# zhaoweicai/mscnn

Hardware: AMD Instinct MI355X
Metric: images/sec mscnn-7s-576 KITTI-car inference (higher is better)
Workload: dtype f32

## Files before the change

include/mscnn_hip.h:

```cpp
#ifndef MSCNN_HIP_H_
#define MSCNN_HIP_H_

#include <stddef.h>
#include <stdint.h>

#if defined(__GNUC__)
#define MSCNN_API __attribute__((visibility("default")))
#else
#define MSCNN_API
#endif

#ifdef __cplusplus
extern "C" {
#endif

typedef enum {
  MSCNN_OK = 0,
  MSCNN_ERR_BAD_ARG = 1,
  MSCNN_ERR_HIP = 2,
  MSCNN_ERR_WORKSPACE = 3,
  MSCNN_ERR_UNSUPPORTED = 4
} mscnn_status;

MSCNN_API const char* mscnn_last_error(void);
MSCNN_API const char* mscnn_version(void);

typedef struct mscnn_conv_plan mscnn_conv_plan;

typedef enum {
  MSCNN_CONV_ALGO_AUTO = 0,
  MSCNN_CONV_ALGO_DIRECT = 1,
  MSCNN_CONV_ALGO_WINO_F2 = 2,
  MSCNN_CONV_ALGO_WINO_F3 = 3,
  MSCNN_CONV_ALGO_F16 = 4,
  MSCNN_CONV_ALGO_WINO_F3_X3 = 5,
  MSCNN_CONV_ALGO_WINO_F4 = 6
} mscnn_conv_algo;

typedef struct {
  int N, Cin, H, W;
  int Cout, Kh, Kw;
  int pad_h, pad_w, stride_h, stride_w, group;
  int relu;
  int algo;
  int tune_variant, tune_grid, tune_flags;
} mscnn_conv_desc;

MSCNN_API int mscnn_conv2d_plan_create(const mscnn_conv_desc* desc, mscnn_conv_plan** plan_out);
MSCNN_API void mscnn_conv2d_plan_destroy(mscnn_conv_plan* plan);
MSCNN_API size_t mscnn_conv2d_packed_weight_bytes(const mscnn_conv_plan* plan);
MSCNN_API size_t mscnn_conv2d_workspace_bytes(const mscnn_conv_plan* plan);
MSCNN_API const char* mscnn_conv2d_plan_kernel(const mscnn_conv_plan* plan);
MSCNN_API double mscnn_conv2d_plan_flops(const mscnn_conv_plan* plan);
MSCNN_API const char* mscnn_conv2d_plan_dtype(const mscnn_conv_plan* plan);
MSCNN_API double mscnn_conv2d_plan_executed_flops(const mscnn_conv_plan* plan);
MSCNN_API int mscnn_conv2d_plan_plane_columns(const mscnn_conv_plan* plan, int* cols, int n);
MSCNN_API int mscnn_conv2d_plan_set_profiling(mscnn_conv_plan* plan, int on);
MSCNN_API int mscnn_conv2d_plan_stage_ms(const mscnn_conv_plan* plan, float ms_out[3]);
#define MSCNN_AMAX_SLOTS 1024
MSCNN_API int mscnn_conv2d_plan_publishes_amax(const mscnn_conv_plan* plan);
MSCNN_API int mscnn_conv2d_plan_set_amax_io(mscnn_conv_plan* plan, const uint32_t* in_bound, uint32_t* out_amax);
MSCNN_API int mscnn_conv2d_plan_set_batch(mscnn_conv_plan* plan, int N);
MSCNN_API unsigned long long mscnn_conv2d_plan_weight_layout(const mscnn_conv_plan* plan);
MSCNN_API int mscnn_conv2d_pack_weights(const mscnn_conv_plan* plan, const float* w, float* packed, void* stream);
MSCNN_API int mscnn_conv2d_fwd_f32(const mscnn_conv_plan* plan, const float* x, const float* w, const float* packed,
                         const float* bias, float* y, void* workspace, size_t workspace_bytes, void* stream);
MSCNN_API int mscnn_conv2d_plan_can_pool(const mscnn_conv_plan* plan);
MSCNN_API int mscnn_conv2d_fwd_pool_f32(const mscnn_conv_plan* plan, const float* x, const float* w, const float* packed,
                              const float* bias, float* y, float* y_pool, void* workspace, size_t workspace_bytes,
                              void* stream);

MSCNN_API int mscnn_relu_fwd_f32(const float* x, float* y, size_t count, float negative_slope, void* stream);

MSCNN_API int mscnn_pool_out_dim(int in, int kernel, int pad, int stride);
MSCNN_API int mscnn_pool2d_fwd_f32(const float* x, float* y, int N, int C, int H, int W, int kernel_h, int kernel_w,
                         int pad_h, int pad_w, int stride_h, int stride_w, int method, void* stream);

MSCNN_API int mscnn_inner_product_fwd_f32(const float* x, const float* w, const float* bias, float* y,
                                int M, int N, int K, int relu, void* stream);
MSCNN_API void mscnn_debug_inner_product_rows(int rows);

MSCNN_API int mscnn_inner_product_wg_supported(int M, int N, int K);
MSCNN_API size_t mscnn_inner_product_wg_packed_bytes(int N, int K);
MSCNN_API size_t mscnn_inner_product_wg_workspace_bytes(int M, int N, int K);
MSCNN_API int mscnn_inner_product_wg_pack(const float* w, float* wt, int N, int K, void* stream);
MSCNN_API int mscnn_inner_product_wg_fwd(const float* x, const float* wt, const float* bias, float* y, int M, int N, int K, int relu,
                                         void* workspace, size_t workspace_bytes, void* stream);
MSCNN_API unsigned long long mscnn_wgemm_handoff_event(void);
MSCNN_API void mscnn_wgemm_force_whole_tiles(int on);
// ... 197 lines not shown
```

mscnn_amd/csrc/conv.hip:

```cpp
#include "common.h"
#include <cstring>
#include "headconv.h"
#include "winograd.h"
#include "wino_x3.h"
#include "wgemm.h"
#include "roipool_wino.h"
#include "wino33_device.h"
#include "conv_c3.h"
#include "wconv.h"
#include "wf2conv.h"
#include "x3_device.h"
#include <new>
#include <type_traits>

namespace {

typedef float f32x16 __attribute__((ext_vector_type(16)));
typedef _Float16 f16x8 __attribute__((ext_vector_type(8)));

struct IgemmArgs {
  const float* x; const float* wp; const float* bias; float* y; float* ws;
  int N, Cin, H, W, Cout, Ho, Wo, pad_h, pad_w;
  int MT, NTH, NTW, NT, KI, G, relu;
  int xcd_map;
// ... 1139 lines not shown
  const int genv = tune_env("MSCNN_TUNE_GRID", d.tune_grid);
  long G = genv > 0 ? genv : ((k.BM == 128 && k.BN == 128 && k.KH == 3 && k.variant != 200) || k.variant == 201 || k.variant == 4 ? 768 : 512);
  if (tiles * p->KI / 4 < G) G = tiles * p->KI / 4;
  if (G < 1) G = 1;
  if (!genv && tiles >= 2 * G) {
    const long tops[3] = {k.variant == 106 ? 1024 : 0, (k.KH == 1 && k.BN == 128 && k.CK < 64) ? 768 : 0, G};
    bool found = false;
    for (int c = 0; c < 3 && !found; ++c)
      for (long g2 = tops[c]; g2 > 0 && g2 >= tops[c] - tops[c] / (k.KH == 3 ? 50 : 16) && g2 * 2 <= tiles; --g2)
        if (tiles % g2 == 0) { G = g2; found = true; break; }
  }
  if (!genv && k.KH == 1 && k.variant >= 101 && tiles >= 256 && tiles <= 768) G = tiles;
  p->G = (int)G;
  p->full_q = (int)(tiles / G);
  p->total_iters = (tiles - (long)p->full_q * G) * p->KI;
  p->packed_bytes = (size_t)p->MT * p->KI * k.KH * k.KW * k.CK * k.BM * ((k.variant >= 200 && k.variant <= 202) ? sizeof(_Float16) : sizeof(float));
  p->ws_bytes = (size_t)p->G * kSlabsPerWg * k.BM * k.BN * sizeof(float);
  if (k.variant == 210) {
    p->x3d_hdr_off = (size_t)p->MT * p->KI * k.KH * k.KW * k.CK * k.BM * 2 * sizeof(_Float16);
    p->packed_bytes = p->x3d_hdr_off + 8192;
    p->x3d_slots_off = p->ws_bytes;
    p->ws_bytes += 4096;
  }
  if (k.KH == 3 && k.KW == 3 && k.BM == 64 && k.CK == 8 && k.RH == 0 && (k.variant == 0 || k.variant == 1) && p->MT == 1 && d.pad_h == 1 &&
      d.pad_w == 1 && !(tune_env("MSCNN_TUNE_FLAGS", d.tune_flags) & 32768)) {
    if (mscnn::wconv_plan(d.N, d.Cin, d.H, d.W, d.Cout, d.tune_variant == 402, &p->wc) && p->wc.packed_bytes == p->packed_bytes) p->wc_use = true;
  }
  if (p->entry >= 0 && k.KH == 3 && k.KW == 3 && k.BM == 64 && k.RH == 0 && (k.variant == 0 || k.variant == 1) && p->MT == 1 && d.pad_h == 1 && d.pad_w == 1 &&
      d.stride_h == 1 && d.stride_w == 1 && d.group == 1 && tune_env("MSCNN_CONV_ALGO", d.algo) == MSCNN_CONV_ALGO_AUTO &&
      !(tune_env("MSCNN_TUNE_FLAGS", d.tune_flags) & 65536) && mscnn::wf2_plan(d.N, d.Cin, d.H, d.W, d.Cout, &p->wf) &&
      (p->wf.tiles >= 512 || d.tune_variant == 403)) {
    p->wf_use = true;
    p->wc_use = false;
    p->packed_bytes = p->wf.packed_bytes;
    p->ws_bytes = 0;
  }
}

extern "C" int mscnn_conv2d_plan_create(const mscnn_conv_desc* desc, mscnn_conv_plan** plan_out) {
  MSCNN_REQUIRE(desc && plan_out, "conv plan: null pointer");
  const mscnn_conv_desc& d = *desc;
  MSCNN_REQUIRE(d.N >= 0 && d.Cin > 0 && d.H > 0 && d.W > 0 && d.Cout > 0 && d.Kh > 0 && d.Kw > 0, "conv plan: bad shape");
  MSCNN_REQUIRE(d.stride_h > 0 && d.stride_w > 0 && d.pad_h >= 0 && d.pad_w >= 0 && d.group > 0, "conv plan: bad params");
  MSCNN_REQUIRE(d.Cin % d.group == 0 && d.Cout % d.group == 0, "conv plan: channels not divisible by group");
  MSCNN_REQUIRE(d.H + 2 * d.pad_h >= d.Kh && d.W + 2 * d.pad_w >= d.Kw, "conv plan: kernel larger than padded input");
  mscnn_conv_plan* p = new (std::nothrow) mscnn_conv_plan();
  MSCNN_REQUIRE(p, "conv plan: out of memory");
  p->d = d;
  plan_shape(p);
  *plan_out = p;
  return MSCNN_OK;
}

extern "C" void mscnn_conv2d_plan_destroy(mscnn_conv_plan* plan) { delete plan; }
extern "C" size_t mscnn_conv2d_packed_weight_bytes(const mscnn_conv_plan* p) { return p ? p->packed_bytes : 0; }
extern "C" size_t mscnn_conv2d_workspace_bytes(const mscnn_conv_plan* p) { return p ? p->ws_bytes : 0; }
extern "C" const char* mscnn_conv2d_plan_kernel(const mscnn_conv_plan* p) {
  if (!p) return "";
  if (p->x3h.rows) return "head_gemm_shiftadd_x3f16";
  if (p->hg) return p->hg_kw ? "head_kwfold_shiftadd_f32" : "head_gemm_shiftadd_f32";
  if (p->head.entry >= 0) return head_kernel_name(p->head);
  if (p->x3.BM) return p->x3.BM == 256 ? "winograd_f3x3_3x3_x3f16_256" : "winograd_f3x3_3x3_x3f16_128";
  if (p->wino) return p->wino_m == 4 ? "winograd_f4x4_3x3" : p->wino_m == 3 ? "winograd_f3x3_3x3" : "winograd_f2x2_3x3";
  if (p->c3) return mscnn::c3_kernel_name();
  if (p->wf_use) return mscnn::wf2_kernel_name();
  if (p->wc_use) return mscnn::wconv_kernel_name();
// ... 38 lines not shown
  const double planes = (double)((p->wino_m + 2) * (p->wino_m + 2)) * (p->x3.BM ? 3.0 : 1.0);
  return 2.0 * planes * d.Cout * d.Cin * ((double)d.N * p->tiles_h * p->tiles_w);
}
extern "C" int mscnn_conv2d_plan_plane_columns(const mscnn_conv_plan* p, int* cols, int n) {
  if (!p || (!p->wino && !p->x3.BM)) return 0;
  const int planes = (p->wino_m + 2) * (p->wino_m + 2);
  for (int i = 0; i < planes && i < n && cols; ++i) cols[i] = p->ragged ? p->wg.cols[i] : p->d.N * p->tiles_h * p->tiles_w;
  return planes;
}
extern "C" long mscnn_debug_wgemm_schedule(const mscnn_conv_plan* p, int whole_tiles, int* rows, long max_rows, int info[8]) {
  if (!p || !p->wino || !p->use_wg) return -1;
  if (info) {
    const int v[8] = {p->wg.tiles, p->wg.MT, p->wg.KI, p->wg.G, p->wg.full_q, p->wg.P, p->wg.BN, p->wg.ragged};
    for (int i = 0; i < 8; ++i) info[i] = v[i];
  }
  return mscnn::wgemm_debug_schedule(p->wg, whole_tiles, rows, max_rows);
}
extern "C" int mscnn_conv2d_plan_set_profiling(mscnn_conv_plan* p, int on) {
  MSCNN_REQUIRE(p, "conv plan: null");
  p->profiling = on != 0;
  p->ev_valid = false;
  if (p->profiling)
    for (hipEvent_t& e : p->ev)
      if (!e) MSCNN_HIP_TRY(hipEventCreate(&e));
  return MSCNN_OK;
}
extern "C" int mscnn_conv2d_plan_stage_ms(const mscnn_conv_plan* p, float ms_out[3]) {
  MSCNN_REQUIRE(p && ms_out, "conv plan: null");
  ms_out[0] = ms_out[1] = ms_out[2] = 0.f;
  MSCNN_REQUIRE(p->profiling && p->ev_valid, "conv plan: no profiled forward yet (mscnn_conv2d_plan_set_profiling)");
  MSCNN_HIP_TRY(hipEventSynchronize(p->ev[3]));
  for (int i = 0; i < 3; ++i) MSCNN_HIP_TRY(hipEventElapsedTime(&ms_out[i], p->ev[i], p->ev[i + 1]));
  return MSCNN_OK;
}
extern "C" int mscnn_conv2d_plan_publishes_amax(const mscnn_conv_plan* p) {
  return p && !p->x3h.rows && (p->x3.BM || (p->wino && p->wino_m >= 3) || p->c3 ||
               (!p->wino && p->head.entry < 0 && p->entry >= 0 && !p->wc_use && !p->wf_use && !(kTable[p->entry].variant >= 200 && kTable[p->entry].variant <= 202))) ? 1 : 0;
}
extern "C" int mscnn_conv2d_plan_set_amax_io(mscnn_conv_plan* p, const uint32_t* in_bound, uint32_t* out_amax) {
  MSCNN_REQUIRE(p, "conv plan: null");
  if (out_amax && !mscnn_conv2d_plan_publishes_amax(p)) {
    set_error("conv plan: kernel %s does not publish max |y|", mscnn_conv2d_plan_kernel(p));
    return MSCNN_ERR_UNSUPPORTED;
  }
  p->amax_in = in_bound;
  p->amax_out = out_amax;
  return MSCNN_OK;
}
extern "C" int mscnn_conv2d_plan_set_batch(mscnn_conv_plan* p, int N) {
  MSCNN_REQUIRE(p && N >= 0, "conv plan: bad batch");
  p->d.N = N;
  plan_shape(p);
  return MSCNN_OK;
}

extern "C" int mscnn_conv2d_pack_weights(const mscnn_conv_plan* p, const float* w, float* packed, void* stream) {
  MSCNN_REQUIRE(p, "conv pack: null plan");
  MSCNN_REQUIRE_ALIGNED(packed, 16, "conv pack: packed");
  if (p->x3h.rows) {
    MSCNN_REQUIRE(w && packed, "conv pack: null pointer");
    return x3_head_pack(p->x3h, w, packed, as_stream(stream));
  }
  if (p->hg) {
    MSCNN_REQUIRE(w && packed, "conv pack: null pointer");
    float* wprime = reinterpret_cast<float*>(reinterpret_cast<unsigned char*>(packed) + p->hg->packed_bytes);
    if (p->hg_kw) {
// ... 386 lines not shown
```

mscnn_amd/csrc/wf2conv.h:

```cpp
#pragma once
#include <hip/hip_runtime.h>
#include <cstddef>

namespace mscnn {

struct Wf2Plan {
  int N, Cin, H, W;
  int NTH, NTW, KI, tiles;
  int cus;
  size_t packed_bytes;
};

bool wf2_plan(int N, int Cin, int H, int W, int Cout, Wf2Plan* out);
const char* wf2_kernel_name();
int wf2_pack(const Wf2Plan& p, const float* w, float* packed, hipStream_t st);
int wf2_launch(const Wf2Plan& p, const float* x, const float* packed, const float* bias, float* y, float* y_pool, int relu, hipStream_t st);

}
```

mscnn_amd/csrc/wf2conv.hip:

```cpp
#include "wf2conv.h"
#include "common.h"
#include <type_traits>

namespace {

typedef float f32x4 __attribute__((ext_vector_type(4)));

struct Wf2Args {
  const float* x; const float* up; const float* bias; float* y; float* yp;
  int N, Cin, H, W, NTH, NTW, KI, relu, tiles;
  int dG_w, dG_h, dG_n;
  unsigned x_bytes;
};

#ifndef WF2_ABL
#define WF2_ABL 0
#endif
#ifdef WF2_TRACE
__device__ unsigned long long g_wf2_trace[2 * 32 * 8];
#define WF2_STAMP(k) do { if (slot == 0 && (wave & 3) == 0 && lane == 0 && u >= 8 && u < 40) g_wf2_trace[((wave >> 2) * 32 + (u - 8)) * 8 + (k)] = __builtin_amdgcn_s_memtime(); } while (0)
#else
#define WF2_STAMP(k) do { } while (0)
#endif
constexpr int TR = 4, TC = 16, NT = TR * TC;
// ... 14 lines not shown
#pragma unroll
  for (int b = 0; b < 3; ++b) {
    const float g0 = g[b], g1 = g[3 + b], g2 = g[6 + b];
    t[0][b] = g0; t[1][b] = 0.5f * (g0 + g1 + g2); t[2][b] = 0.5f * (g0 - g1 + g2); t[3][b] = g2;
  }
#pragma unroll
  for (int a = 0; a < 4; ++a) {
    const float u0 = t[a][0], u1 = 0.5f * (t[a][0] + t[a][1] + t[a][2]), u2 = 0.5f * (t[a][0] - t[a][1] + t[a][2]), u3 = t[a][2];
    *reinterpret_cast<float4*>(up + (((long)ci * 4 + a) * 64 + co) * 4) = make_float4(u0, u1, u2, u3);
  }
}

__device__ __forceinline__ __amdgpu_buffer_rsrc_t make_rsrc(const void* p, unsigned bytes) {
  return __builtin_amdgcn_make_buffer_rsrc(const_cast<void*>(p), 0, (int)bytes, 0x00020000);
}
constexpr unsigned kOob = 0x80000000u;
__device__ __forceinline__ void dma16(__amdgpu_buffer_rsrc_t rsrc, unsigned voff, unsigned soff, unsigned lds_addr) {
  soff = __builtin_amdgcn_readfirstlane(soff);
  lds_addr = __builtin_amdgcn_readfirstlane(lds_addr);
  asm volatile("s_nop 4\n\ts_mov_b32 m0, %3\n\ts_nop 0\n\tbuffer_load_dwordx4 %0, %1, %2 offen lds" ::"v"(voff), "s"(rsrc), "s"(soff), "s"(lds_addr) : "memory");
}
__device__ __forceinline__ void dma4(__amdgpu_buffer_rsrc_t rsrc, unsigned voff, unsigned soff, unsigned lds_addr) {
  soff = __builtin_amdgcn_readfirstlane(soff);
  lds_addr = __builtin_amdgcn_readfirstlane(lds_addr);
  asm volatile("s_nop 4\n\ts_mov_b32 m0, %3\n\ts_nop 0\n\tbuffer_load_dword %0, %1, %2 offen lds" ::"v"(voff), "s"(rsrc), "s"(soff), "s"(lds_addr) : "memory");
}
__device__ __forceinline__ void dma_wait() { asm volatile("s_waitcnt vmcnt(0)" ::: "memory"); }

constexpr int P_PIECES = (P_FLOATS + 255) / 256;
constexpr int P_SLOTS = (P_PIECES + 7) / 8;
constexpr int LDS_SPARE = LDS_FLOATS * 4;
static_assert(LDS_SPARE + 1024 + 256 <= 160 * 1024, "LDS");

__global__ __launch_bounds__(512, 2) void wf2conv_kernel(Wf2Args a) {
  __shared__ __attribute__((aligned(1024))) float lds[LDS_FLOATS + 256 + 64];
  float* const Us = lds;
  float* const Vs = lds + 2 * U_FLOATS;
  float* const Ps = lds + 2 * U_FLOATS + 2 * V_FLOATS;
  const unsigned lds0 = (unsigned)(size_t)lds;
  const int tid = threadIdx.x, lane = tid & 63;
  const int wave = __builtin_amdgcn_readfirstlane(tid >> 6);
  const int l16 = lane & 15, lq = lane >> 4;
  const int ch = wave & 1, tr = wave >> 1;
  const bool mfma_first = wave >= 4;
  const int HW = a.H * a.W;
  const int G = (int)gridDim.x, slot = (int)blockIdx.x;
  const int my_tiles = slot < a.tiles ? (a.tiles - slot + G - 1) / G : 0;
  const int total = my_tiles * a.KI;
  if (total == 0) return;
  const __amdgpu_buffer_rsrc_t rU = make_rsrc(a.up, (unsigned)(a.KI * U_FLOATS * 4)), rX = make_rsrc(a.x, a.x_bytes);

  unsigned vP[P_SLOTS];
#pragma unroll
  for (int j = 0; j < P_SLOTS; ++j) vP[j] = kOob;
  int p_tw = slot % a.NTW, p_th = (slot / a.NTW) % a.NTH, p_n = slot / (a.NTW * a.NTH);
  unsigned p_img = 0;
  int pu = 0;
  auto enter_tile = [&]() {
    const int h0 = p_th * (2 * TR), w0 = p_tw * (2 * TC);
    p_img = __builtin_amdgcn_readfirstlane((unsigned)(p_n * a.Cin) * (unsigned)HW * 4u);
#pragma unroll
    for (int j = 0; j < P_SLOTS; ++j) {
      const int f = (wave + 8 * j) * 64 + lane;
      const int k = f / (PR * PC4), rem = f - k * (PR * PC4), r = rem / PC4, c4 = rem - r * PC4;
      const int hh = h0 - 1 + r, ww = w0 - 4 + 4 * c4;
      const bool ok = f < P_FLOATS / 4 && (unsigned)hh < (unsigned)a.H && (unsigned)ww < (unsigned)a.W;
      vP[j] = ok ? (unsigned)(k * HW + hh * a.W + ww) * 4u : kOob;
    }
    p_tw += a.dG_w; if (p_tw >= a.NTW) { p_tw -= a.NTW; ++p_th; }
    p_th += a.dG_h; if (p_th >= a.NTH) { p_th -= a.NTH; ++p_n; }
    p_n += a.dG_n;
  };
  auto dma_patch = [&](int buf) {
    if (pu < total) {
      const int kc = pu % a.KI;
      if (kc == 0) enter_tile();
      const unsigned sb = p_img + (unsigned)(kc * CK) * (unsigned)HW * 4u;
      const unsigned pb = lds0 + (unsigned)((2 * U_FLOATS + 2 * V_FLOATS + buf * P_STRIDE) * 4);
#pragma unroll
      for (int j = 0; j < P_SLOTS; ++j) {
        const int piece = wave + 8 * j;
        dma16(rX, vP[j], sb, piece < P_PIECES ? pb + (unsigned)piece * 1024u : lds0 + (unsigned)LDS_SPARE);
      }
    }
    ++pu;
  };
  auto dma_u = [&](int kc, int stage) {
    const unsigned ub = lds0 + (unsigned)(stage * U_FLOATS * 4);
#pragma unroll
    for (int j = 0; j < 4; ++j) {
      const unsigned piece = (unsigned)(wave * 4 + j);
      dma16(rU, (unsigned)lane * 16u, (unsigned)kc * (U_FLOATS * 4) + piece * 1024u, ub + piece * 1024u);
    }
  };
  auto transform = [&](int buf, int stage) {
    const int trn = lane >> 4, tcn = lane & 15;
    const float* p = Ps + buf * P_STRIDE + wave * (PR * PC) + (2 * trn) * PC + PX + 2 * tcn;
    float d[4][4];
#pragma unroll
    for (int i = 0; i < 4; ++i)
#pragma unroll
      for (int j = 0; j < 4; ++j) d[i][j] = p[i * PC + j];
    float t[4][4];
#pragma unroll
    for (int j = 0; j < 4; ++j) {
      t[0][j] = d[0][j] - d[2][j]; t[1][j] = d[1][j] + d[2][j]; t[2][j] = d[2][j] - d[1][j]; t[3][j] = d[1][j] - d[3][j];
    }
    float4* V = reinterpret_cast<float4*>(Vs + stage * V_FLOATS);
#pragma unroll
    for (int i = 0; i < 4; ++i)
      V[(wave * 4 + i) * NT + lane] = make_float4(t[i][0] - t[i][2], t[i][1] + t[i][2], t[i][2] - t[i][1], t[i][1] - t[i][3]);
  };

  f32x4 acc[16][2];

  auto mfmas = [&](int st, int c, auto first_c) {
    constexpr bool FIRST = decltype(first_c)::value;
    const f32x4* U = reinterpret_cast<const f32x4*>(Us + st * U_FLOATS) + lq * 4 * 64 + ch * 32 + l16;
    const f32x4* V = reinterpret_cast<const f32x4*>(Vs + st * V_FLOATS) + lq * 4 * NT + tr * 16 + l16;
    f32x4 a0[2], a1[2], bb[2];
    auto rd = [&](int g, int buf) {
      const int off = ((g >> 2) * 16 + (g & 3)) * 64;
      if (WF2_ABL & 2) { a0[buf] = (f32x4){1.f, 2.f, 3.f, (float)c}; a1[buf] = a0[buf]; bb[buf] = a0[buf]; }
      else { a0[buf] = U[off]; a1[buf] = U[off + 16]; bb[buf] = V[off]; }
    };
    rd(0, 0);
#pragma unroll
    for (int g = 0; g < 8; ++g) {
      const int cur = g & 1, i = g & 3;
      if (g + 1 < 8) rd(g + 1, cur ^ 1);
      __builtin_amdgcn_sched_barrier(0);
      if (WF2_ABL & 1) { acc[i * 4][0][0] = (FIRST && g == 0 ? 0.f : acc[i * 4][0][0]) + a0[cur][0] + a1[cur][1] + bb[cur][2]; continue; }
#pragma unroll
      for (int q = 0; q < 4; ++q) {
        const bool fresh = FIRST && g < 4;
        acc[i * 4 + q][0] = __builtin_amdgcn_mfma_f32_16x16x4f32(a0[cur][q], bb[cur][q], fresh ? (f32x4){0.f, 0.f, 0.f, 0.f} : acc[i * 4 + q][0], 0, 0, 0);
        acc[i * 4 + q][1] = __builtin_amdgcn_mfma_f32_16x16x4f32(a1[cur][q], bb[cur][q], fresh ? (f32x4){0.f, 0.f, 0.f, 0.f} : acc[i * 4 + q][1], 0, 0, 0);
      }
      __builtin_amdgcn_sched_barrier(0);
    }
  };

  const int Hp = a.H / 2, Wp = a.W / 2;
  int c_tw = slot % a.NTW, c_th = (slot / a.NTW) % a.NTH, c_n = slot / (a.NTW * a.NTH);
  float* const bias_s = lds + LDS_FLOATS + 256;
  if (tid < 64) bias_s[tid] = a.bias ? a.bias[tid] : 0.f;
  auto epilogue = [&]() {
    const int oh = c_th * (2 * TR) + 2 * tr, ow = c_tw * (2 * TC) + 2 * l16;
    const long co0 = (long)c_n * 64 + ch * 32 + lq * 4;
    float* ydst = a.y ? a.y + (co0 * a.H + oh) * a.W + ow : nullptr;
    float* pdst = a.yp ? a.yp + (co0 * Hp + (oh >> 1)) * Wp + (ow >> 1) : nullptr;
#pragma unroll
    for (int mb = 0; mb < 2; ++mb)
#pragma unroll
      for (int r = 0; r < 4; ++r) {
        float s0[4], s1[4];
#pragma unroll
        for (int j = 0; j < 4; ++j) {
          const float m0 = acc[0 + j][mb][r], m1 = acc[4 + j][mb][r], m2 = acc[8 + j][mb][r], m3 = acc[12 + j][mb][r];
          s0[j] = m0 + m1 + m2;
          s1[j] = m1 - m2 - m3;
        }
        const float bv = bias_s[ch * 32 + mb * 16 + lq * 4 + r];
        const long cofs = (long)(mb * 16 + r);
        if (!ydst) {
          const float q00 = s0[0] + s0[1] + s0[2], q01 = s0[1] - s0[2] - s0[3], q10 = s1[0] + s1[1] + s1[2], q11 = s1[1] - s1[2] - s1[3];
          float m = q00;
          if (q01 > m) m = q01;
          if (q10 > m) m = q10;
          if (q11 > m) m = q11;
          m += bv;
          if (a.relu) m = m < 0.f ? 0.f : m;
          pdst[cofs * (Hp * Wp)] = m;
          continue;
        }
        float y00 = s0[0] + s0[1] + s0[2] + bv, y01 = s0[1] - s0[2] - s0[3] + bv;
        float y10 = s1[0] + s1[1] + s1[2] + bv, y11 = s1[1] - s1[2] - s1[3] + bv;
        if (a.relu) {
          y00 = y00 < 0.f ? 0.f : y00; y01 = y01 < 0.f ? 0.f : y01; y10 = y10 < 0.f ? 0.f : y10; y11 = y11 < 0.f ? 0.f : y11;
        }
        if (ydst) {
          float* dst = ydst + cofs * HW;
          *reinterpret_cast<float2*>(dst) = make_float2(y00, y01);
          *reinterpret_cast<float2*>(dst + a.W) = make_float2(y10, y11);
        }
        if (pdst) {
          float m = y00;
          if (y01 > m) m = y01;
          if (y10 > m) m = y10;
          if (y11 > m) m = y11;
          pdst[cofs * (Hp * Wp)] = m;
        }
      }
    c_tw += a.dG_w; if (c_tw >= a.NTW) { c_tw -= a.NTW; ++c_th; }
    c_th += a.dG_h; if (c_th >= a.NTH) { c_th -= a.NTH; ++c_n; }
    c_n += a.dG_n;
  };

  dma_u(0, 0);
  dma_patch(0);
  dma_patch(1);
  dma_wait();
  __syncthreads();
  transform(0, 0);
  __syncthreads();

  for (int u = 0; u < total; ++u) {
    const int st = u & 1, c = u % a.KI;
    const bool more1 = u + 1 < total;
    WF2_STAMP(0);
    if (!mfma_first) {
      if (!(WF2_ABL & 8)) {
        dma_u(c + 1 < a.KI ? c + 1 : 0, st ^ 1);
        dma_patch(st);
      }
      if (more1 && !(WF2_ABL & 4)) transform(st ^ 1, st ^ 1);
    }
    WF2_STAMP(1);
    if (c == 0) mfmas(st, c, std::true_type{});
    else mfmas(st, c, std::false_type{});
    WF2_STAMP(2);
    if (c == a.KI - 1) epilogue();
    WF2_STAMP(3);
    if (mfma_first) {
      if (!(WF2_ABL & 8)) {
        dma_u(c + 1 < a.KI ? c + 1 : 0, st ^ 1);
        dma_patch(st);
      }
      if (more1 && !(WF2_ABL & 4)) transform(st ^ 1, st ^ 1);
    }
    WF2_STAMP(4);
    dma_wait();
    if (!(WF2_ABL & 16)) __syncthreads();
    WF2_STAMP(5);
  }
}

}

namespace mscnn {

bool wf2_plan(int N, int Cin, int H, int W, int Cout, Wf2Plan* o) {
  if (Cout != 64 || Cin % CK != 0 || Cin < CK || N < 1 || H % (2 * TR) != 0 || W % (2 * TC) != 0) return false;
  if ((double)N * (Cin > 64 ? Cin : 64) * H * W * 4.0 >= 2147483648.0 - 65536.0) return false;
  o->N = N; o->Cin = Cin; o->H = H; o->W = W;
  o->NTH = H / (2 * TR); o->NTW = W / (2 * TC); o->KI = Cin / CK;
  o->tiles = N * o->NTH * o->NTW;
  o->packed_bytes = (size_t)16 * 64 * Cin * sizeof(float);
  int dev = 0, cus = 0;
  if (hipGetDevice(&dev) != hipSuccess || hipDeviceGetAttribute(&cus, hipDeviceAttributeMultiprocessorCount, dev) != hipSuccess || cus <= 0) {
    (void)hipGetLastError();
    cus = 256;
  }
  o->cus = cus;
  return true;
}

const char* wf2_kernel_name() { return "winograd2x2_fused_k3x3_c64"; }

int wf2_pack(const Wf2Plan& p, const float* w, float* packed, hipStream_t st) {
  wf2_weight_kernel<<<cdiv(64 * p.Cin, 256), 256, 0, st>>>(w, packed, p.Cin);
  MSCNN_POST_LAUNCH();
  return MSCNN_OK;
}

int wf2_launch(const Wf2Plan& p, const float* x, const float* packed, const float* bias, float* y, float* y_pool, int relu, hipStream_t st) {
  MSCNN_REQUIRE(x && packed && (y || y_pool), "conv(winograd2x2 fused): null pointer");
  MSCNN_REQUIRE(reinterpret_cast<uintptr_t>(packed) % 16 == 0 && reinterpret_cast<uintptr_t>(x) % 16 == 0 && (!y || reinterpret_cast<uintptr_t>(y) % 8 == 0),
                "conv(winograd2x2 fused): x and the packed weights must be 16-byte, y 8-byte aligned");
  Wf2Args a;
  a.x = x; a.up = packed; a.bias = bias; a.y = y; a.yp = y_pool;
  a.N = p.N; a.Cin = p.Cin; a.H = p.H; a.W = p.W; a.NTH = p.NTH; a.NTW = p.NTW; a.KI = p.KI; a.relu = relu; a.tiles = p.tiles;
  const int cus = p.cus;
  const int G = p.tiles < cus ? p.tiles : cus;
  a.dG_w = G % p.NTW; a.dG_h = (G / p.NTW) % p.NTH; a.dG_n = G / (p.NTW * p.NTH);
  a.x_bytes = (unsigned)((size_t)p.N * p.Cin * p.H * p.W * sizeof(float));
  wf2conv_kernel<<<G, 512, 0, st>>>(a);
  MSCNN_POST_LAUNCH();
  return MSCNN_OK;
}

}

#ifdef WF2_TRACE
extern "C" __attribute__((visibility("default"))) int mscnn_debug_wf2_trace(unsigned long long* host_out) {
  return (int)hipMemcpyFromSymbol(host_out, HIP_SYMBOL(g_wf2_trace), sizeof(unsigned long long) * 2 * 32 * 8);
}
#endif
```

mscnn_amd/hipapi.py:

```python
import ctypes as C
import os

import numpy as np
import torch

_HERE = os.path.dirname(os.path.abspath(__file__))
LIB_PATH = os.path.join(_HERE, "libmscnn_hip.so")
_lib = None


class MscnnError(RuntimeError):
    pass


class ConvDesc(C.Structure):
    _fields_ = [(n, C.c_int) for n in ("N", "Cin", "H", "W", "Cout", "Kh", "Kw", "pad_h", "pad_w",
                                       "stride_h", "stride_w", "group", "relu", "algo", "tune_variant", "tune_grid", "tune_flags")]


AMAX_SLOTS = 1024
ALGO_AUTO, ALGO_DIRECT, ALGO_WINO_F2, ALGO_WINO_F3, ALGO_F16, ALGO_WINO_F3_X3, ALGO_WINO_F4 = 0, 1, 2, 3, 4, 5, 6


MAX_HEADS = 16
# ... 67 lines not shown
        L.mscnn_inner_product_x3_packed_bytes.argtypes = [C.c_int, C.c_int]
        L.mscnn_inner_product_x3_workspace_bytes.restype = C.c_size_t
        L.mscnn_inner_product_x3_workspace_bytes.argtypes = [C.c_int] * 3
        L.mscnn_inner_product_x3_pack.argtypes = [C.c_void_p, C.c_void_p, C.c_int, C.c_int, C.c_void_p]
        L.mscnn_inner_product_x3_fwd.argtypes = [C.c_void_p] * 4 + [C.c_int] * 4 + [C.c_void_p, C.c_void_p, C.c_size_t, C.c_void_p]
        L.mscnn_inner_product_wg_supported.argtypes = [C.c_int] * 3
        L.mscnn_inner_product_wg_packed_bytes.restype = C.c_size_t
        L.mscnn_inner_product_wg_packed_bytes.argtypes = [C.c_int, C.c_int]
        L.mscnn_inner_product_wg_workspace_bytes.restype = C.c_size_t
        L.mscnn_inner_product_wg_workspace_bytes.argtypes = [C.c_int] * 3
        L.mscnn_inner_product_wg_pack.argtypes = [C.c_void_p, C.c_void_p, C.c_int, C.c_int, C.c_void_p]
        L.mscnn_inner_product_wg_fwd.argtypes = [C.c_void_p] * 4 + [C.c_int] * 4 + [C.c_void_p, C.c_size_t, C.c_void_p]
        L.mscnn_max_rel_diff_f32.argtypes = [C.c_void_p, C.c_void_p, C.c_size_t, C.c_float, C.c_void_p, C.c_void_p]
        L.mscnn_sum_squares_f32.argtypes = [C.c_void_p, C.c_size_t, C.c_void_p, C.c_void_p]
        L.mscnn_max_rel_diff_strided_f32.argtypes = [C.c_void_p, C.c_size_t, C.c_void_p, C.c_size_t, C.c_size_t, C.c_size_t, C.c_void_p, C.c_double,
                                                     C.c_void_p, C.c_void_p]
        L.mscnn_store_words_i32.argtypes = [C.c_void_p, C.c_void_p, C.c_int, C.c_void_p]
        L.mscnn_wgemm_handoff_event.restype = C.c_ulonglong
        L.mscnn_wgemm_handoff_event.argtypes = []
        L.mscnn_wgemm_force_whole_tiles.restype = None
        L.mscnn_wgemm_force_whole_tiles.argtypes = [C.c_int]
        L.mscnn_wgemm_whole_tiles_forced.argtypes = []
        L.mscnn_debug_inner_product_rows.restype = None
        L.mscnn_debug_inner_product_rows.argtypes = [C.c_int]
        L.mscnn_debug_wgemm_handoff_fault.restype = None
        L.mscnn_debug_wgemm_handoff_fault.argtypes = [C.c_int, C.c_uint]
        L.mscnn_inner_product_pack_f16.argtypes = [C.c_void_p, C.c_void_p, C.c_int, C.c_int, C.c_void_p]
        L.mscnn_inner_product_fwd_f16.argtypes = [C.c_void_p] * 4 + [C.c_int] * 4 + [C.c_void_p]
        for f in ("mscnn_conv2d_plan_flops", "mscnn_conv2d_plan_executed_flops"):
            getattr(L, f).restype = C.c_double
            getattr(L, f).argtypes = [C.c_void_p]
        L.mscnn_conv2d_plan_set_profiling.argtypes = [C.c_void_p, C.c_int]
        L.mscnn_conv2d_plan_plane_columns.argtypes = [C.c_void_p, C.c_void_p, C.c_int]
        L.mscnn_debug_wgemm_schedule.restype = C.c_long
        L.mscnn_debug_wgemm_schedule.argtypes = [C.c_void_p, C.c_int, C.c_void_p, C.c_long, C.c_void_p]
        L.mscnn_conv2d_plan_stage_ms.argtypes = [C.c_void_p, C.c_void_p]
        for f in ("mscnn_conv2d_packed_weight_bytes", "mscnn_conv2d_workspace_bytes"):
            getattr(L, f).restype = C.c_size_t
            getattr(L, f).argtypes = [C.c_void_p]
        L.mscnn_conv2d_plan_destroy.argtypes = [C.c_void_p]
        L.mscnn_conv2d_plan_destroy.restype = None
        L.mscnn_conv2d_plan_set_batch.argtypes = [C.c_void_p, C.c_int]
        L.mscnn_conv2d_pack_weights.argtypes = [C.c_void_p] * 4
        L.mscnn_conv2d_fwd_f32.argtypes = [C.c_void_p] * 7 + [C.c_size_t, C.c_void_p]
        L.mscnn_conv2d_fwd_pool_f32.argtypes = [C.c_void_p] * 8 + [C.c_size_t, C.c_void_p]
        L.mscnn_conv2d_plan_can_pool.argtypes = [C.c_void_p]
        L.mscnn_conv2d_plan_can_fuse_roipool.argtypes = [C.c_void_p, C.c_int, C.c_int, C.c_int]
        L.mscnn_conv2d_plan_can_chain.argtypes = [C.c_void_p, C.c_void_p]
        L.mscnn_conv2d_plan_can_pool_only.argtypes = [C.c_void_p]
        L.mscnn_conv2d_fwd_chain_f32.argtypes = [C.c_void_p] * 8 + [C.c_size_t, C.c_void_p, C.c_size_t, C.c_void_p]
        L.mscnn_conv2d_roipool_workspace_bytes.restype = C.c_size_t
        L.mscnn_conv2d_roipool_workspace_bytes.argtypes = [C.c_void_p] + [C.c_int] * 4
        L.mscnn_conv2d_fwd_roipool_pair_f32.argtypes = ([C.c_void_p, C.c_void_p, C.c_void_p] + [C.c_int] * 4 + [C.c_void_p, C.c_float, C.c_float, C.c_float]
                                                        + [C.c_void_p] * 4 + [C.c_size_t, C.c_void_p])
        L.mscnn_roipool_maps_bytes.restype = C.c_size_t
        L.mscnn_roipool_maps_bytes.argtypes = [C.c_int] * 4
        L.mscnn_roipool_maps_build_f32.argtypes = [C.c_void_p, C.c_void_p] + [C.c_int] * 4 + [C.c_void_p]
        L.mscnn_conv2d_plan_weight_layout.argtypes = [C.c_void_p]
        L.mscnn_conv2d_plan_weight_layout.restype = C.c_ulonglong
        L.mscnn_relu_fwd_f32.argtypes = [C.c_void_p, C.c_void_p, C.c_size_t, C.c_float, C.c_void_p]
        L.mscnn_pool2d_fwd_f32.argtypes = [C.c_void_p, C.c_void_p] + [C.c_int] * 11 + [C.c_void_p]
        L.mscnn_inner_product_fwd_f32.argtypes = [C.c_void_p] * 4 + [C.c_int] * 4 + [C.c_void_p]
        L.mscnn_concat_channels_f32.argtypes = [C.c_void_p, C.c_void_p] + [C.c_int] * 5 + [C.c_void_p]
        L.mscnn_deconv_depthwise_fwd_f32.argtypes = [C.c_void_p] * 4 + [C.c_int] * 10 + [C.c_void_p]
        L.mscnn_softmax_fwd_f32.argtypes = [C.c_void_p, C.c_void_p, C.c_int, C.c_int, C.c_int, C.c_void_p]
        L.mscnn_roipool_fwd_f32.argtypes = ([C.c_void_p] * 3 + [C.c_int] * 7 + [C.c_float, C.c_float] + [C.c_int] * 2
# ... 119 lines not shown
        rows = np.zeros((max(n, 1), 7), dtype=np.int32)
        got = lib().mscnn_debug_wgemm_schedule(self._p, int(bool(whole_tiles)), rows.ctypes.data_as(C.c_void_p), n, info)
        assert got == n
        keys = ("tiles", "MT", "KI", "G", "full_q", "planes", "BN", "ragged")
        return {k: int(info[i]) for i, k in enumerate(keys)}, rows[:n]

    def set_profiling(self, on=True):
        _check(lib().mscnn_conv2d_plan_set_profiling(self._p, int(on)))

    def stage_ms(self):
        out = (C.c_float * 3)()
        _check(lib().mscnn_conv2d_plan_stage_ms(self._p, out))
        return tuple(out)

    def out_shape(self):
        d = self.desc
        return (d.N, d.Cout, (d.H + 2 * d.pad_h - d.Kh) // d.stride_h + 1, (d.W + 2 * d.pad_w - d.Kw) // d.stride_w + 1)

    def set_batch(self, N):
        before, had = lib().mscnn_conv2d_plan_weight_layout(self._p), self.packed
        _check(lib().mscnn_conv2d_plan_set_batch(self._p, N))
        self.desc.N = N
        self._alloc()
        if getattr(self, "w", None) is not None and self.packed is not None and \
                (lib().mscnn_conv2d_plan_weight_layout(self._p) != before or self.packed is not had):
            self.pack(self.w)

    def pack(self, w):
        self.w = w
        if self.packed is not None:
            _check(lib().mscnn_conv2d_pack_weights(self._p, _dev(w), _dev(self.packed), _stream()))

    @property
    def publishes_amax(self):
        return bool(lib().mscnn_conv2d_plan_publishes_amax(self._p))

    def set_amax_io(self, in_bound=None, out_amax=None):
        self._amax = (in_bound, out_amax)
        _check(lib().mscnn_conv2d_plan_set_amax_io(self._p, _dev(in_bound), _dev(out_amax)))

    @property
    def can_pool(self):
        return bool(lib().mscnn_conv2d_plan_can_pool(self._p))

    def forward(self, x, bias=None, out=None, pool_out=None):
        if out is None:
            out = torch.empty(self.out_shape(), dtype=torch.float32, device=x.device)
        wsb = self.ws.numel() * 4 if self.ws is not None else 0
        _check(lib().mscnn_conv2d_fwd_pool_f32(self._p, _dev(x), _dev(self.w), _dev(self.packed), _dev(bias), _dev(out),
                                               _dev(pool_out), _dev(self.ws), wsb, _stream()))
        return out

    @property
    def can_pool_only(self):
        return bool(lib().mscnn_conv2d_plan_can_pool_only(self._p))

    def can_chain(self, nxt):
        return bool(lib().mscnn_conv2d_plan_can_chain(self._p, nxt._p))

    def forward_chain(self, x, nxt, bias=None, out=None, pool_out=None, write_y=True):
        if out is None and write_y:
            out = torch.empty(self.out_shape(), dtype=torch.float32, device=self.ws.device)
        wsb = self.ws.numel() * 4
        _check(lib().mscnn_conv2d_fwd_chain_f32(self._p, nxt._p if nxt is not None else None, _dev(x), _dev(self.packed), _dev(bias),
                                                _dev(out) if write_y else None, _dev(pool_out), _dev(self.ws), wsb,
                                                _dev(nxt.ws) if nxt is not None else None, nxt.ws.numel() * 4 if nxt is not None else 0,
# ... 516 lines not shown
```

Measured before the change: 228.9.

## Interleave DMA and input transform into MFMA groups in Winograd F2 conv kernel

Adds a templated schedule variant of the wf2conv kernel, enabled by default. It issues the next stage's U and patch DMA pieces between the MFMAs of the first group, and spreads the Winograd input transform of the next buffer across MFMA groups, using sched_group_barrier pinning and register laundering. This is meant to hide LDS reads, transform ALU work and DMA issue latency behind matrix instructions instead of running them as separate phases. It also makes the epilogue use 32-bit offsets, and a tune flag falls back to the old schedule. In exchange it raises register pressure and makes correctness depend on the interleaved ordering.

```diff
diff --git a/include/mscnn_hip.h b/include/mscnn_hip.h
--- a/include/mscnn_hip.h
+++ b/include/mscnn_hip.h
@@ -55,6 +55,7 @@
 MSCNN_API const char* mscnn_conv2d_plan_dtype(const mscnn_conv_plan* plan);
 MSCNN_API double mscnn_conv2d_plan_executed_flops(const mscnn_conv_plan* plan);
 MSCNN_API int mscnn_conv2d_plan_plane_columns(const mscnn_conv_plan* plan, int* cols, int n);
+MSCNN_API int mscnn_conv2d_plan_wave_schedule(const mscnn_conv_plan* plan);
 MSCNN_API int mscnn_conv2d_plan_set_profiling(mscnn_conv_plan* plan, int on);
 MSCNN_API int mscnn_conv2d_plan_stage_ms(const mscnn_conv_plan* plan, float ms_out[3]);
 #define MSCNN_AMAX_SLOTS 1024
diff --git a/mscnn_amd/csrc/conv.hip b/mscnn_amd/csrc/conv.hip
--- a/mscnn_amd/csrc/conv.hip
+++ b/mscnn_amd/csrc/conv.hip
@@ -1195,6 +1195,7 @@
       (p->wf.tiles >= 512 || d.tune_variant == 403)) {
     p->wf_use = true;
     p->wc_use = false;
+    if (tune_env("MSCNN_TUNE_FLAGS", d.tune_flags) & 262144) p->wf.sched = 0;
     p->packed_bytes = p->wf.packed_bytes;
     p->ws_bytes = 0;
   }
@@ -1299,6 +1300,9 @@
   MSCNN_HIP_TRY(hipEventSynchronize(p->ev[3]));
   for (int i = 0; i < 3; ++i) MSCNN_HIP_TRY(hipEventElapsedTime(&ms_out[i], p->ev[i], p->ev[i + 1]));
   return MSCNN_OK;
+}
+extern "C" int mscnn_conv2d_plan_wave_schedule(const mscnn_conv_plan* p) {
+  return p && p->wf_use ? p->wf.sched : -1;
 }
 extern "C" int mscnn_conv2d_plan_publishes_amax(const mscnn_conv_plan* p) {
   return p && !p->x3h.rows && (p->x3.BM || (p->wino && p->wino_m >= 3) || p->c3 ||
diff --git a/mscnn_amd/csrc/wf2conv.h b/mscnn_amd/csrc/wf2conv.h
--- a/mscnn_amd/csrc/wf2conv.h
+++ b/mscnn_amd/csrc/wf2conv.h
@@ -8,6 +8,7 @@
   int N, Cin, H, W;
   int NTH, NTW, KI, tiles;
   int cus;
+  int sched;
   size_t packed_bytes;
 };
 
diff --git a/mscnn_amd/csrc/wf2conv.hip b/mscnn_amd/csrc/wf2conv.hip
--- a/mscnn_amd/csrc/wf2conv.hip
+++ b/mscnn_amd/csrc/wf2conv.hip
@@ -70,6 +70,10 @@
 constexpr int LDS_SPARE = LDS_FLOATS * 4;
 static_assert(LDS_SPARE + 1024 + 256 <= 160 * 1024, "LDS");
 
+template <int TAG, typename T>
+__device__ __forceinline__ void launder(T& v) { asm volatile("" : "+v"(v) : "n"(TAG)); }
+
+template <int SCHED>
 __global__ __launch_bounds__(512, 2) void wf2conv_kernel(Wf2Args a) {
   __shared__ __attribute__((aligned(1024))) float lds[LDS_FLOATS + 256 + 64];
   float* const Us = lds;
@@ -94,7 +98,7 @@
   int p_tw = slot % a.NTW, p_th = (slot / a.NTW) % a.NTH, p_n = slot / (a.NTW * a.NTH);
   unsigned p_img = 0;
   int pu = 0;
-  auto enter_tile = [&]() {
+  auto enter_tile = [&]() __attribute__((always_inline)) {
     const int h0 = p_th * (2 * TR), w0 = p_tw * (2 * TC);
     p_img = __builtin_amdgcn_readfirstlane((unsigned)(p_n * a.Cin) * (unsigned)HW * 4u);
 #pragma unroll
@@ -109,7 +113,7 @@
     p_th += a.dG_h; if (p_th >= a.NTH) { p_th -= a.NTH; ++p_n; }
     p_n += a.dG_n;
   };
-  auto dma_patch = [&](int buf) {
+  auto dma_patch = [&](int buf) __attribute__((always_inline)) {
     if (pu < total) {
       const int kc = pu % a.KI;
       if (kc == 0) enter_tile();
@@ -123,7 +127,7 @@
     }
     ++pu;
   };
-  auto dma_u = [&](int kc, int stage) {
+  auto dma_u = [&](int kc, int stage) __attribute__((always_inline)) {
     const unsigned ub = lds0 + (unsigned)(stage * U_FLOATS * 4);
 #pragma unroll
     for (int j = 0; j < 4; ++j) {
@@ -131,7 +135,30 @@
       dma16(rU, (unsigned)lane * 16u, (unsigned)kc * (U_FLOATS * 4) + piece * 1024u, ub + piece * 1024u);
     }
   };
-  auto transform = [&](int buf, int stage) {
+  unsigned d_us = 0, d_ub = 0, d_sb = 0, d_pb = 0;
+  bool d_live = false;
+  auto dma_prep = [&](int c, int st) __attribute__((always_inline)) {
+    d_us = (unsigned)(c + 1 < a.KI ? c + 1 : 0) * (U_FLOATS * 4);
+    d_ub = lds0 + (unsigned)((st ^ 1) * U_FLOATS * 4);
+    d_live = pu < total;
+    const int kc = pu % a.KI;
+    if (d_live && kc == 0) enter_tile();
+    d_sb = p_img + (unsigned)(kc * CK) * (unsigned)HW * 4u;
+    d_pb = lds0 + (unsigned)((2 * U_FLOATS + 2 * V_FLOATS + st * P_STRIDE) * 4);
+    ++pu;
+  };
+  auto dma_piece = [&](int m) __attribute__((always_inline)) {
+    __builtin_amdgcn_sched_barrier(0);
+    if (m < 4) {
+      const unsigned piece = (unsigned)(wave * 4 + m);
+      dma16(rU, (unsigned)lane * 16u, d_us + piece * 1024u, d_ub + piece * 1024u);
+    } else {
+      const int piece = wave + 8 * (m - 4);
+      dma16(rX, d_live ? vP[m - 4] : kOob, d_sb, piece < P_PIECES ? d_pb + (unsigned)piece * 1024u : lds0 + (unsigned)LDS_SPARE);
+    }
+    __builtin_amdgcn_sched_barrier(0);
+  };
+  auto transform = [&](int buf, int stage) __attribute__((always_inline)) {
     const int trn = lane >> 4, tcn = lane & 15;
     const float* p = Ps + buf * P_STRIDE + wave * (PR * PC) + (2 * trn) * PC + PX + 2 * tcn;
     float d[4][4];
@@ -150,14 +177,60 @@
       V[(wave * 4 + i) * NT + lane] = make_float4(t[i][0] - t[i][2], t[i][1] + t[i][2], t[i][2] - t[i][1], t[i][1] - t[i][3]);
   };
 
+  float xd[4][4], xt[4][4];
+  unsigned xo = 0;
+  float4* xV = nullptr;
+  auto fill = [&](int s, auto tag_c) __attribute__((always_inline)) {
+    constexpr int TAG = decltype(tag_c)::value;
+    if (WF2_ABL & 4) return;
+    if (s == 0) {
+      unsigned o = xo;
+      launder<TAG>(o);
+      const float* p = lds + o;
+#pragma unroll
+      for (int i = 0; i < 4; ++i)
+#pragma unroll
+        for (int j = 0; j < 4; ++j) xd[i][j] = p[i * PC + j];
+    } else if (s == 1 || s == 2) {
+#pragma unroll
+      for (int j = 2 * (s - 1); j < 2 * (s - 1) + 2; ++j) {
+        xt[0][j] = xd[0][j] - xd[2][j]; xt[1][j] = xd[1][j] + xd[2][j]; xt[2][j] = xd[2][j] - xd[1][j]; xt[3][j] = xd[1][j] - xd[3][j];
+#pragma unroll
+        for (int i = 0; i < 4; ++i) launder<TAG>(xt[i][j]);
+      }
+    } else if (s == 3 || s == 4) {
+#pragma unroll
+      for (int i = 2 * (s - 3); i < 2 * (s - 3) + 2; ++i) {
+        xd[i][0] = xt[i][0] - xt[i][2]; xd[i][1] = xt[i][1] + xt[i][2]; xd[i][2] = xt[i][2] - xt[i][1]; xd[i][3] = xt[i][1] - xt[i][3];
+#pragma unroll
+        for (int j = 0; j < 4; ++j) launder<TAG>(xd[i][j]);
+      }
+    } else if (s == 5) {
+#pragma unroll
+      for (int i = 0; i < 4; ++i) xV[(wave * 4 + i) * NT + lane] = make_float4(xd[i][0], xd[i][1], xd[i][2], xd[i][3]);
+    }
+  };
+  auto pin = [&](int s) __attribute__((always_inline)) {
+    if ((WF2_ABL & 4) || s < 0 || s > 5) return;
+    __builtin_amdgcn_sched_group_barrier(0x100, 3, 0);
+#pragma unroll
+    for (int q = 0; q < 8; ++q) {
+      __builtin_amdgcn_sched_group_barrier(0x8, 1, 0);
+      if (s == 0) __builtin_amdgcn_sched_group_barrier(0x100, 1, 0);
+      else if (s < 5) __builtin_amdgcn_sched_group_barrier(0x2, 1, 0);
+      else if (q & 1) __builtin_amdgcn_sched_group_barrier(0x200, 1, 0);
+    }
+  };
+
   f32x4 acc[16][2];
 
-  auto mfmas = [&](int st, int c, auto first_c) {
+  auto mfmas = [&](int st, int c, auto first_c, auto slot0_c, auto dgroup_c) __attribute__((always_inline)) {
     constexpr bool FIRST = decltype(first_c)::value;
+    constexpr int SLOT0 = decltype(slot0_c)::value, DGROUP = decltype(dgroup_c)::value;
     const f32x4* U = reinterpret_cast<const f32x4*>(Us + st * U_FLOATS) + lq * 4 * 64 + ch * 32 + l16;
     const f32x4* V = reinterpret_cast<const f32x4*>(Vs + st * V_FLOATS) + lq * 4 * NT + tr * 16 + l16;
     f32x4 a0[2], a1[2], bb[2];
-    auto rd = [&](int g, int buf) {
+    auto rd = [&](int g, int buf) __attribute__((always_inline)) {
       const int off = ((g >> 2) * 16 + (g & 3)) * 64;
       if (WF2_ABL & 2) { a0[buf] = (f32x4){1.f, 2.f, 3.f, (float)c}; a1[buf] = a0[buf]; bb[buf] = a0[buf]; }
       else { a0[buf] = U[off]; a1[buf] = U[off + 16]; bb[buf] = V[off]; }
@@ -167,14 +240,27 @@
     for (int g = 0; g < 8; ++g) {
       const int cur = g & 1, i = g & 3;
       if (g + 1 < 8) rd(g + 1, cur ^ 1);
-      __builtin_amdgcn_sched_barrier(0);
-      if (WF2_ABL & 1) { acc[i * 4][0][0] = (FIRST && g == 0 ? 0.f : acc[i * 4][0][0]) + a0[cur][0] + a1[cur][1] + bb[cur][2]; continue; }
+      const int s = SLOT0 < 0 ? -1 : g - SLOT0;
+      const bool filled = !(WF2_ABL & 4) && s >= 0 && s <= 5;
+      if (filled) fill(s, std::integral_constant<int, 2 * SLOT0 + FIRST>{});
+      else __builtin_amdgcn_sched_barrier(0);
+      if (WF2_ABL & 1) {
+        acc[i * 4][0][0] = (FIRST && g == 0 ? 0.f : acc[i * 4][0][0]) + a0[cur][0] + a1[cur][1] + bb[cur][2];
+        if (g == DGROUP && !(WF2_ABL & 8))
+#pragma unroll
+          for (int m = 0; m < 6; ++m) dma_piece(m);
+        __builtin_amdgcn_sched_barrier(0);
+        continue;
+      }
 #pragma unroll
       for (int q = 0; q < 4; ++q) {
         const bool fresh = FIRST && g < 4;
         acc[i * 4 + q][0] = __builtin_amdgcn_mfma_f32_16x16x4f32(a0[cur][q], bb[cur][q], fresh ? (f32x4){0.f, 0.f, 0.f, 0.f} : acc[i * 4 + q][0], 0, 0, 0);
+        if (g == DGROUP && q < 3 && !(WF2_ABL & 8)) dma_piece(2 * q);
         acc[i * 4 + q][1] = __builtin_amdgcn_mfma_f32_16x16x4f32(a1[cur][q], bb[cur][q], fresh ? (f32x4){0.f, 0.f, 0.f, 0.f} : acc[i * 4 + q][1], 0, 0, 0);
-      }
+        if (g == DGROUP && q < 3 && !(WF2_ABL & 8)) dma_piece(2 * q + 1);
+      }
+      if (filled) pin(s);
       __builtin_amdgcn_sched_barrier(0);
     }
   };
@@ -183,11 +269,13 @@
   int c_tw = slot % a.NTW, c_th = (slot / a.NTW) % a.NTH, c_n = slot / (a.NTW * a.NTH);
   float* const bias_s = lds + LDS_FLOATS + 256;
   if (tid < 64) bias_s[tid] = a.bias ? a.bias[tid] : 0.f;
-  auto epilogue = [&]() {
+  const bool has_y = a.y != nullptr, has_p = a.yp != nullptr;
+  auto epilogue = [&]() __attribute__((always_inline)) {
     const int oh = c_th * (2 * TR) + 2 * tr, ow = c_tw * (2 * TC) + 2 * l16;
-    const long co0 = (long)c_n * 64 + ch * 32 + lq * 4;
-    float* ydst = a.y ? a.y + (co0 * a.H + oh) * a.W + ow : nullptr;
-    float* pdst = a.yp ? a.yp + (co0 * Hp + (oh >> 1)) * Wp + (ow >> 1) : nullptr;
+    const int co0 = ch * 32 + lq * 4;
+    float* const ybase = a.y + (long)c_n * 64 * HW;
+    float* const pbase = a.yp + (long)c_n * 64 * (Hp * Wp);
+    const unsigned yofs = (unsigned)((co0 * a.H + oh) * a.W + ow), pofs = (unsigned)((co0 * Hp + (oh >> 1)) * Wp + (ow >> 1));
 #pragma unroll
     for (int mb = 0; mb < 2; ++mb)
 #pragma unroll
@@ -200,8 +288,8 @@
           s1[j] = m1 - m2 - m3;
         }
         const float bv = bias_s[ch * 32 + mb * 16 + lq * 4 + r];
-        const long cofs = (long)(mb * 16 + r);
-        if (!ydst) {
+        const unsigned cofs = (unsigned)(mb * 16 + r);
+        if (!has_y) {
           const float q00 = s0[0] + s0[1] + s0[2], q01 = s0[1] - s0[2] - s0[3], q10 = s1[0] + s1[1] + s1[2], q11 = s1[1] - s1[2] - s1[3];
           float m = q00;
           if (q01 > m) m = q01;
@@ -209,7 +297,7 @@
           if (q11 > m) m = q11;
           m += bv;
           if (a.relu) m = m < 0.f ? 0.f : m;
-          pdst[cofs * (Hp * Wp)] = m;
+          pbase[pofs + cofs * (unsigned)(Hp * Wp)] = m;
           continue;
         }
         float y00 = s0[0] + s0[1] + s0[2] + bv, y01 = s0[1] - s0[2] - s0[3] + bv;
@@ -217,17 +305,17 @@
         if (a.relu) {
           y00 = y00 < 0.f ? 0.f : y00; y01 = y01 < 0.f ? 0.f : y01; y10 = y10 < 0.f ? 0.f : y10; y11 = y11 < 0.f ? 0.f : y11;
         }
-        if (ydst) {
-          float* dst = ydst + cofs * HW;
+        if (has_y) {
+          float* dst = ybase + (yofs + cofs * (unsigned)HW);
           *reinterpret_cast<float2*>(dst) = make_float2(y00, y01);
           *reinterpret_cast<float2*>(dst + a.W) = make_float2(y10, y11);
         }
-        if (pdst) {
+        if (has_p) {
           float m = y00;
           if (y01 > m) m = y01;
           if (y10 > m) m = y10;
           if (y11 > m) m = y11;
-          pdst[cofs * (Hp * Wp)] = m;
+          pbase[pofs + cofs * (unsigned)(Hp * Wp)] = m;
         }
       }
     c_tw += a.dG_w; if (c_tw >= a.NTW) { c_tw -= a.NTW; ++c_th; }
@@ -243,31 +331,46 @@
   transform(0, 0);
   __syncthreads();
 
+  const std::integral_constant<int, SCHED ? 0 : -1> dgroup_c;
+  const std::integral_constant<int, SCHED ? 1 : -1> slot0_c;
   for (int u = 0; u < total; ++u) {
     const int st = u & 1, c = u % a.KI;
     const bool more1 = u + 1 < total;
     WF2_STAMP(0);
-    if (!mfma_first) {
-      if (!(WF2_ABL & 8)) {
-        dma_u(c + 1 < a.KI ? c + 1 : 0, st ^ 1);
-        dma_patch(st);
-      }
-      if (more1 && !(WF2_ABL & 4)) transform(st ^ 1, st ^ 1);
-    }
-    WF2_STAMP(1);
-    if (c == 0) mfmas(st, c, std::true_type{});
-    else mfmas(st, c, std::false_type{});
-    WF2_STAMP(2);
-    if (c == a.KI - 1) epilogue();
-    WF2_STAMP(3);
-    if (mfma_first) {
-      if (!(WF2_ABL & 8)) {
-        dma_u(c + 1 < a.KI ? c + 1 : 0, st ^ 1);
-        dma_patch(st);
-      }
-      if (more1 && !(WF2_ABL & 4)) transform(st ^ 1, st ^ 1);
-    }
-    WF2_STAMP(4);
+    if constexpr (SCHED == 0) {
+      if (!mfma_first) {
+        if (!(WF2_ABL & 8)) {
+          dma_u(c + 1 < a.KI ? c + 1 : 0, st ^ 1);
+          dma_patch(st);
+        }
+        if (more1 && !(WF2_ABL & 4)) transform(st ^ 1, st ^ 1);
+      }
+      WF2_STAMP(1);
+      if (c == 0) mfmas(st, c, std::true_type{}, slot0_c, dgroup_c);
+      else mfmas(st, c, std::false_type{}, slot0_c, dgroup_c);
+      WF2_STAMP(2);
+      if (c == a.KI - 1) epilogue();
+      WF2_STAMP(3);
+      if (mfma_first) {
+        if (!(WF2_ABL & 8)) {
+          dma_u(c + 1 < a.KI ? c + 1 : 0, st ^ 1);
+          dma_patch(st);
+        }
+        if (more1 && !(WF2_ABL & 4)) transform(st ^ 1, st ^ 1);
+      }
+      WF2_STAMP(4);
+    } else {
+      if (!(WF2_ABL & 8)) dma_prep(c, st);
+      WF2_STAMP(1);
+      xo = (unsigned)(2 * U_FLOATS + 2 * V_FLOATS + (st ^ 1) * P_STRIDE + wave * (PR * PC) + (2 * (lane >> 4)) * PC + PX + 2 * (lane & 15));
+      xV = reinterpret_cast<float4*>(Vs + (st ^ 1) * V_FLOATS);
+      if (c == 0) mfmas(st, c, std::true_type{}, slot0_c, dgroup_c);
+      else mfmas(st, c, std::false_type{}, slot0_c, dgroup_c);
+      WF2_STAMP(2);
+      if (c == a.KI - 1) epilogue();
+      WF2_STAMP(3);
+      WF2_STAMP(4);
+    }
     dma_wait();
     if (!(WF2_ABL & 16)) __syncthreads();
     WF2_STAMP(5);
@@ -291,6 +394,7 @@
     cus = 256;
   }
   o->cus = cus;
+  o->sched = 1;
   return true;
 }
 
@@ -313,7 +417,8 @@
   const int G = p.tiles < cus ? p.tiles : cus;
   a.dG_w = G % p.NTW; a.dG_h = (G / p.NTW) % p.NTH; a.dG_n = G / (p.NTW * p.NTH);
   a.x_bytes = (unsigned)((size_t)p.N * p.Cin * p.H * p.W * sizeof(float));
-  wf2conv_kernel<<<G, 512, 0, st>>>(a);
+  if (p.sched == 0) wf2conv_kernel<0><<<G, 512, 0, st>>>(a);
+  else wf2conv_kernel<1><<<G, 512, 0, st>>>(a);
   MSCNN_POST_LAUNCH();
   return MSCNN_OK;
 }
diff --git a/mscnn_amd/hipapi.py b/mscnn_amd/hipapi.py
--- a/mscnn_amd/hipapi.py
+++ b/mscnn_amd/hipapi.py
@@ -123,6 +123,7 @@
             getattr(L, f).argtypes = [C.c_void_p]
         L.mscnn_conv2d_plan_set_profiling.argtypes = [C.c_void_p, C.c_int]
         L.mscnn_conv2d_plan_plane_columns.argtypes = [C.c_void_p, C.c_void_p, C.c_int]
+        L.mscnn_conv2d_plan_wave_schedule.argtypes = [C.c_void_p]
         L.mscnn_debug_wgemm_schedule.restype = C.c_long
         L.mscnn_debug_wgemm_schedule.argtypes = [C.c_void_p, C.c_int, C.c_void_p, C.c_long, C.c_void_p]
         L.mscnn_conv2d_plan_stage_ms.argtypes = [C.c_void_p, C.c_void_p]
@@ -308,6 +309,10 @@
             _check(lib().mscnn_conv2d_pack_weights(self._p, _dev(w), _dev(self.packed), _stream()))
 
     @property
+    def wave_schedule(self):
+        return int(lib().mscnn_conv2d_plan_wave_schedule(self._p))
+
+    @property
     def publishes_amax(self):
         return bool(lib().mscnn_conv2d_plan_publishes_amax(self._p))
 
```

New measurement: 231.0, median of 6. About the same (+0.9%).
